# bifurcation/fourq

Hardware: NVIDIA B200
Metric: curve4q_variable_base_dh_scalar_mults_per_s (higher is better)
Workload: dtype u32

## Files before the change

### fourq_b200/csrc/fp.cuh

```cuda
#pragma once
#include "arith.cuh"

struct fp { u32 v[4]; };

struct fpb { u32 b0, b1, b2, b3, e1, e2, e3, d2, d3; };

struct facc { u32 e0, e1, e2, e3, e4, o1, o2, o3, o4, o5; };

struct fpw { u32 w[6]; };

#define FQ_P3 0x7fffffffu

FQ_FN fp fp_set(u32 a0, u32 a1, u32 a2, u32 a3) { fp r; r.v[0] = a0; r.v[1] = a1; r.v[2] = a2; r.v[3] = a3; return r; }
FQ_FN fp fp_zero() { return fp_set(0, 0, 0, 0); }
FQ_FN fp fp_one() { return fp_set(1, 0, 0, 0); }


FQ_FN fp fp_add_loose(const fp& a, const fp& b) {
  fp r;
  r.v[0] = add_cc(a.v[0], b.v[0]); r.v[1] = addc_cc(a.v[1], b.v[1]);
  r.v[2] = addc_cc(a.v[2], b.v[2]); r.v[3] = addc(a.v[3], b.v[3]);
  return r;
}

FQ_FN fp fp_fold1(const fp& x) {
  fp r; u32 t = x.v[3] >> 31;
  r.v[0] = add_cc(x.v[0], t); r.v[1] = addc_cc(x.v[1], 0);
  r.v[2] = addc_cc(x.v[2], 0); r.v[3] = addc(x.v[3] & FQ_P3, 0);
  return r;
}

FQ_FN fp fp_add(const fp& a, const fp& b) { return fp_fold1(fp_add_loose(a, b)); }

FQ_FN fp fp_sub(const fp& a, const fp& b) {
  fp r;
  r.v[0] = sub_cc(a.v[0], b.v[0]); r.v[1] = subc_cc(a.v[1], b.v[1]);
  r.v[2] = subc_cc(a.v[2], b.v[2]); r.v[3] = subc_cc(a.v[3], b.v[3]);
  r.v[0] = subc_cc(r.v[0], 0); r.v[1] = subc_cc(r.v[1], 0);
  r.v[2] = subc_cc(r.v[2], 0); r.v[3] = subc(r.v[3], 0) & FQ_P3;
  return r;
}

FQ_FN fp fp_neg(const fp& a) { return fp_set(~a.v[0], ~a.v[1], ~a.v[2], a.v[3] ^ FQ_P3); }

FQ_FN fp fp_dbl(const fp& a) {
  return fp_set((a.v[0] << 1) | (a.v[3] >> 30), shl_pair(a.v[0], a.v[1], 1), shl_pair(a.v[1], a.v[2], 1),
                shl_pair(a.v[2], a.v[3], 1) & FQ_P3);
}
FQ_FN fp fp_half(const fp& a) {
  return fp_set(shr_pair(a.v[0], a.v[1], 1), shr_pair(a.v[1], a.v[2], 1), shr_pair(a.v[2], a.v[3], 1),
                (a.v[3] >> 1) | ((a.v[0] & 1) << 30));
}

FQ_FN fp fp_canon(const fp& a) {
  u32 allones = a.v[0] & a.v[1] & a.v[2] & (a.v[3] | 0x80000000u);
  u32 m = (allones == 0xffffffffu) ? 0u : 0xffffffffu;
  return fp_set(a.v[0] & m, a.v[1] & m, a.v[2] & m, a.v[3] & m);
}
FQ_FN bool fp_eq_canon(const fp& a, const fp& b) {
  return ((a.v[0] ^ b.v[0]) | (a.v[1] ^ b.v[1]) | (a.v[2] ^ b.v[2]) | (a.v[3] ^ b.v[3])) == 0;
}
FQ_FN bool fp_is_zero(const fp& a) {
  u32 o = a.v[0] | a.v[1] | a.v[2] | a.v[3];
  u32 n = a.v[0] & a.v[1] & a.v[2] & (a.v[3] | 0x80000000u);
  return (o == 0) | (n == 0xffffffffu);
}
FQ_FN fp fp_select(u32 m, const fp& x, const fp& y) {
  return fp_set(y.v[0] ^ (m & (x.v[0] ^ y.v[0])), y.v[1] ^ (m & (x.v[1] ^ y.v[1])),
                y.v[2] ^ (m & (x.v[2] ^ y.v[2])), y.v[3] ^ (m & (x.v[3] ^ y.v[3])));
}
FQ_FN fp fp_from_u128(const fp& x) { return fp_fold1(fp_fold1(x)); }


FQ_FN fpb fp_prep(const fp& b) {
  fpb B;
  B.b0 = b.v[0]; B.b1 = b.v[1]; B.b2 = b.v[2]; B.b3 = b.v[3];
  B.e1 = b.v[1] << 1; B.e2 = b.v[2] << 1; B.e3 = b.v[3] << 1;
  B.d2 = shl_pair(b.v[1], b.v[2], 1); B.d3 = shl_pair(b.v[2], b.v[3], 1);
  return B;
}

FQ_FN void facc_zero(facc& A) { A.e0 = A.e1 = A.e2 = A.e3 = A.e4 = A.o1 = A.o2 = A.o3 = A.o4 = A.o5 = 0; }

template <int K> FQ_FN void facc_init_kp(facc& A) {
  A.e0 = 0; A.e1 = 0u - (1u << (K - 32)); A.e2 = 0xffffffffu; A.e3 = 0xffffffffu; A.e4 = 0;
  A.o1 = 0; A.o2 = 0; A.o3 = 0; A.o4 = 0xffffffffu; A.o5 = (1u << (K - 33)) - 1u;
}

FQ_FN void facc_row0(facc& A, u32 a, u32 v0, u32 v1, u32 v2, u32 v3) {
  mul_wide(A.e0, A.e1, a, v0); mul_wide(A.e2, A.e3, a, v2); A.e4 = 0;
  mul_wide(A.o1, A.o2, a, v1); mul_wide(A.o3, A.o4, a, v3); A.o5 = 0;
}
FQ_FN void facc_row(facc& A, u32 a, u32 v0, u32 v1, u32 v2, u32 v3) {
  A.e0 = mad_lo_cc(a, v0, A.e0); A.e1 = madc_hi_cc(a, v0, A.e1);
  A.e2 = madc_lo_cc(a, v2, A.e2); A.e3 = madc_hi_cc(a, v2, A.e3); A.e4 = addc(A.e4, 0);
  A.o1 = mad_lo_cc(a, v1, A.o1); A.o2 = madc_hi_cc(a, v1, A.o2);
  A.o3 = madc_lo_cc(a, v3, A.o3); A.o4 = madc_hi_cc(a, v3, A.o4); A.o5 = addc(A.o5, 0);
}

template <bool FRESH> FQ_FN void facc_mul(facc& A, const fp& a, const fpb& B) {
  if (FRESH) facc_row0(A, a.v[0], B.b0, B.b1, B.b2, B.b3);
  else facc_row(A, a.v[0], B.b0, B.b1, B.b2, B.b3);
  facc_row(A, a.v[1], B.e3, B.b0, B.b1, B.b2);
  facc_row(A, a.v[2], B.e2, B.d3, B.b0, B.b1);
  facc_row(A, a.v[3], B.e1, B.d2, B.d3, B.b0);
}

FQ_FN fpw facc_merge(const facc& A) {
  fpw r;
  r.w[0] = A.e0; r.w[1] = add_cc(A.e1, A.o1); r.w[2] = addc_cc(A.e2, A.o2); r.w[3] = addc_cc(A.e3, A.o3);
  r.w[4] = addc_cc(A.e4, A.o4); r.w[5] = addc(A.o5, 0);
  return r;
}
FQ_FN fpw fpw_add(const fpw& a, const fpw& b) {
  fpw r;
  r.w[0] = add_cc(a.w[0], b.w[0]); r.w[1] = addc_cc(a.w[1], b.w[1]); r.w[2] = addc_cc(a.w[2], b.w[2]);
  r.w[3] = addc_cc(a.w[3], b.w[3]); r.w[4] = addc_cc(a.w[4], b.w[4]); r.w[5] = addc(a.w[5], b.w[5]);
  return r;
}
FQ_FN fpw fpw_sub(const fpw& a, const fpw& b) {
  fpw r;
  r.w[0] = sub_cc(a.w[0], b.w[0]); r.w[1] = subc_cc(a.w[1], b.w[1]); r.w[2] = subc_cc(a.w[2], b.w[2]);
  r.w[3] = subc_cc(a.w[3], b.w[3]); r.w[4] = subc_cc(a.w[4], b.w[4]); r.w[5] = subc(a.w[5], b.w[5]);
  return r;
}

FQ_FN fp fp_fold(const fpw& x) {
  fp r;
  u32 tlo = shr_pair(x.w[3], x.w[4], 31), thi = shr_pair(x.w[4], x.w[5], 31);
  r.v[0] = add_cc(x.w[0], tlo); r.v[1] = addc_cc(x.w[1], thi);
  r.v[2] = addc_cc(x.w[2], 0); r.v[3] = addc(x.w[3] & FQ_P3, 0);
  u32 top = r.v[3] >> 31;
  r.v[3] &= FQ_P3;
  r.v[0] = add_cc(r.v[0], top); r.v[1] = addc(r.v[1], 0);
  return r;
}

FQ_FN fp fp_mul_prep(const fp& a, const fpb& B) {
  facc A; facc_mul<true>(A, a, B);
  return fp_fold(facc_merge(A));
}
FQ_FN fp fp_mul(const fp& a, const fp& b) { return fp_mul_prep(a, fp_prep(b)); }
FQ_FN fp fp_fold7(u32 w0, u32 w1, u32 w2, u32 w3, u32 w4, u32 w5, u32 w6) {
  fp r;
  u32 t0 = shr_pair(w3, w4, 31), t1 = shr_pair(w4, w5, 31), t2 = shr_pair(w5, w6, 31), t3 = w6 >> 31;
  r.v[0] = add_cc(w0, t0); r.v[1] = addc_cc(w1, t1); r.v[2] = addc_cc(w2, t2); r.v[3] = addc(w3 & FQ_P3, t3);
  u32 top = r.v[3] >> 31;
  r.v[3] &= FQ_P3;
  r.v[0] = add_cc(r.v[0], top); r.v[1] = addc_cc(r.v[1], 0); r.v[2] = addc_cc(r.v[2], 0); r.v[3] = addc(r.v[3], 0);
  return r;
}
FQ_FN fp fp_sqr(const fp& a) {
  const u32 a0 = a.v[0], a1 = a.v[1], a2 = a.v[2], a3 = a.v[3];
  const u32 e1 = a1 << 1, e2 = a2 << 1, e3 = a3 << 1, d2 = shl_pair(a1, a2, 1), d3 = shl_pair(a2, a3, 1);
  u32 E0, E1, E2, E3, E4, E5, E6, O1, O2, O3, O4, O5, O6;
  mul_wide(E0, E1, a0, a0); mul_wide(E2, E3, a0, d2); mul_wide(E4, E5, a1, d3);
  E2 = mad_lo_cc(a1, a1, E2); E3 = madc_hi_cc(a1, a1, E3); E4 = madc_lo_cc(a2, a2, E4); E5 = madc_hi_cc(a2, a2, E5); E6 = addc(0, 0);
  E2 = mad_lo_cc(a3, e3, E2); E3 = madc_hi_cc(a3, e3, E3); E4 = addc_cc(E4, 0); E5 = addc_cc(E5, 0); E6 = addc(E6, 0);
  mul_wide(O1, O2, a0, e1); mul_wide(O3, O4, a0, d3); mul_wide(O5, O6, a2, e3);
  O3 = mad_lo_cc(a1, e2, O3); O4 = madc_hi_cc(a1, e2, O4); O5 = addc_cc(O5, 0); O6 = addc(O6, 0);
  u32 w1 = add_cc(E1, O1), w2 = addc_cc(E2, O2), w3 = addc_cc(E3, O3), w4 = addc_cc(E4, O4), w5 = addc_cc(E5, O5), w6 = addc(E6, O6);
  return fp_fold7(E0, w1, w2, w3, w4, w5, w6);
}

FQ_FN fp fp_nsqr(fp x, int n) {
  FQ_NOUNROLL
  for (int i = 0; i < n; i++) x = fp_sqr(x);
  return x;
}

FQ_FN fp fp_inv(const fp& x) {
  fp x3 = fp_mul(fp_sqr(x), x);
  fp xf = fp_mul(fp_nsqr(x3, 2), x3);
  fp x8 = fp_mul(fp_nsqr(xf, 4), xf);
  fp x16 = fp_mul(fp_nsqr(x8, 8), x8);
  fp x32 = fp_mul(fp_nsqr(x16, 16), x16);
  fp t = fp_mul(fp_nsqr(x32, 32), x32);
  t = fp_mul(fp_nsqr(t, 32), x32);
  t = fp_mul(fp_nsqr(t, 16), x16);
  t = fp_mul(fp_nsqr(t, 8), x8);
  t = fp_mul(fp_nsqr(t, 4), xf);
  t = fp_mul(fp_sqr(t), x);
  return fp_mul(fp_nsqr(t, 2), x);
}

FQ_FN fp fp_invsqrt(const fp& x) {
  fp x3 = fp_mul(fp_sqr(x), x);
  fp xf = fp_mul(fp_nsqr(x3, 2), x3);
  fp x5 = fp_mul(fp_sqr(xf), x);
  fp x10 = fp_mul(fp_nsqr(x5, 5), x5);
  fp x20 = fp_mul(fp_nsqr(x10, 10), x10);
  fp x25 = fp_mul(fp_nsqr(x20, 5), x5);
  fp x50 = fp_mul(fp_nsqr(x25, 25), x25);
  fp x100 = fp_mul(fp_nsqr(x50, 50), x50);
  fp x125 = fp_mul(fp_nsqr(x100, 25), x25);
  return x125;
}
```

### fourq_b200/csrc/fp2.cuh

```cuda
#pragma once
#include "fp.cuh"

struct fp2 { fp re, im; };

struct fp2b { fpb re, im, sum; };

FQ_FN fp2 fp2_set(const fp& re, const fp& im) { fp2 r; r.re = re; r.im = im; return r; }
FQ_FN fp2 fp2_zero() { return fp2_set(fp_zero(), fp_zero()); }
FQ_FN fp2 fp2_one() { return fp2_set(fp_one(), fp_zero()); }

FQ_FN fp2 fp2_add(const fp2& a, const fp2& b) { return fp2_set(fp_add(a.re, b.re), fp_add(a.im, b.im)); }
FQ_FN fp2 fp2_sub(const fp2& a, const fp2& b) { return fp2_set(fp_sub(a.re, b.re), fp_sub(a.im, b.im)); }
FQ_FN fp2 fp2_neg(const fp2& a) { return fp2_set(fp_neg(a.re), fp_neg(a.im)); }
FQ_FN fp2 fp2_conj(const fp2& a) { return fp2_set(a.re, fp_neg(a.im)); }
FQ_FN fp2 fp2_dbl(const fp2& a) { return fp2_set(fp_dbl(a.re), fp_dbl(a.im)); }
FQ_FN fp2 fp2_canon(const fp2& a) { return fp2_set(fp_canon(a.re), fp_canon(a.im)); }
FQ_FN bool fp2_eq_canon(const fp2& a, const fp2& b) { return fp_eq_canon(a.re, b.re) & fp_eq_canon(a.im, b.im); }
FQ_FN bool fp2_eq(const fp2& a, const fp2& b) { return fp2_eq_canon(fp2_canon(a), fp2_canon(b)); }
FQ_FN fp2 fp2_select(u32 m, const fp2& x, const fp2& y) { return fp2_set(fp_select(m, x.re, y.re), fp_select(m, x.im, y.im)); }

#ifdef FQ_FP2_SCHOOLBOOK
FQ_FN fp2b fp2_prep(const fp2& b) {
  fp2b B;
  B.re = fp_prep(b.re); B.im = fp_prep(b.im); B.sum = B.re;
  return B;
}
FQ_FN fp2 fp2_mul_prep(const fp2& a, const fp2b& B) {
  facc A0, A1;
  facc_mul<true>(A0, a.re, B.re); facc_mul<false>(A0, fp_neg(a.im), B.im);
  facc_mul<true>(A1, a.re, B.im); facc_mul<false>(A1, a.im, B.re);
  fp2 r;
  r.re = fp_fold(facc_merge(A0));
  r.im = fp_fold(facc_merge(A1));
  return r;
}
#else
FQ_FN fp2b fp2_prep(const fp2& b) {
  fp2b B;
  B.re = fp_prep(b.re); B.im = fp_prep(b.im); B.sum = fp_prep(fp_add(b.re, b.im));
  return B;
}

FQ_FN fp2 fp2_mul_prep(const fp2& a, const fp2b& B) {
  facc A0, A1, A2;
  facc_init_kp<36>(A0); facc_mul<false>(A0, a.re, B.re);
  facc_mul<true>(A1, a.im, B.im);
  facc_init_kp<38>(A2); facc_mul<false>(A2, fp_add_loose(a.re, a.im), B.sum);
  fpw t0 = facc_merge(A0), t1 = facc_merge(A1), t2 = facc_merge(A2);
  fp2 r;
  r.re = fp_fold(fpw_sub(t0, t1));
  r.im = fp_fold(fpw_sub(fpw_sub(t2, t0), t1));
  return r;
}
#endif
FQ_FN fp2 fp2_mul(const fp2& a, const fp2& b) { return fp2_mul_prep(a, fp2_prep(b)); }

FQ_FN fp2 fp2_sqr(const fp2& a) {
  fp2 r;
  r.re = fp_mul_prep(fp_add_loose(a.re, a.im), fp_prep(fp_sub(a.re, a.im)));
  r.im = fp_mul_prep(fp_add_loose(a.re, a.re), fp_prep(a.im));
  return r;
}

FQ_FN fp2 fp2_inv(const fp2& a) {
  fp n = fp_inv(fp_add(fp_sqr(a.re), fp_sqr(a.im)));
  fpb N = fp_prep(n);
  return fp2_set(fp_mul_prep(a.re, N), fp_mul_prep(fp_neg(a.im), N));
}

#ifdef FQ_HOSTSIM
#define FQ_CALL static inline
#else
#define FQ_CALL static __device__ __noinline__
#endif
FQ_CALL fp2 fp2_mul_c(fp2 a, fp2 b) { return fp2_mul(a, b); }
FQ_CALL fp2 fp2_sqr_c(fp2 a) { return fp2_sqr(a); }
FQ_CALL fp fp_invsqrt_c(fp a) { return fp_invsqrt(a); }
```

### fourq_b200/csrc/point.cuh

```cuda
#pragma once
#include "fp2.cuh"

struct ptR1 { fp2 X, Y, Z, Ta, Tb; };
struct ptR2 { fp2 N, D, E, F; };
struct ptR3p { fp2b N, D, E, F; };

FQ_FN fp2 curve_d() { return fp2_set(fp_set(0x00000142u, 0x00000000u, 0x000000e4u, 0x00000000u), fp_set(0xf1fc0c8du, 0xb3821488u, 0x6657e0fcu, 0x5e472f84u)); }
FQ_FN fp2 curve_2d() { return fp2_set(fp_set(0x00000284u, 0x00000000u, 0x000001c8u, 0x00000000u), fp_set(0xe3f8191bu, 0x67042911u, 0xccafc1f9u, 0x3c8e5f08u)); }
FQ_FN fp2 curve_gx() { return fp2_set(fp_set(0x7b3833aau, 0x286592adu, 0x7c2fb305u, 0x1a347223u), fp_set(0x60ac77f6u, 0x96869fb3u, 0x2878aa9cu, 0x1e1f553fu)); }
FQ_FN fp2 curve_gy() { return fp2_set(fp_set(0x2bcbb287u, 0xb924a246u, 0xa120785au, 0x0e3fee9bu), fp_set(0x844c8b5cu, 0x49a7c344u, 0x630e0242u, 0x6e1c4af8u)); }

FQ_CALL bool pt_on_curve(fp2 x, fp2 y) {
  fp2 x2 = fp2_sqr_c(x), y2 = fp2_sqr_c(y);
  fp2 lhs = fp2_sub(y2, x2);
  fp2 rhs = fp2_add(fp2_one(), fp2_mul_c(fp2_mul_c(curve_d(), x2), y2));
  return fp2_eq(lhs, rhs);
}

FQ_FN ptR1 pt_from_affine(const fp2& x, const fp2& y) { ptR1 P; P.X = x; P.Y = y; P.Z = fp2_one(); P.Ta = x; P.Tb = y; return P; }

FQ_FN ptR2 pt_r1_to_r2(const ptR1& P) {
  ptR2 R;
  R.N = fp2_add(P.X, P.Y); R.D = fp2_sub(P.Y, P.X); R.E = fp2_dbl(P.Z);
  R.F = fp2_mul(fp2_mul(P.Ta, P.Tb), curve_2d());
  return R;
}
FQ_FN ptR3p pt_r1_to_r3p(const ptR1& P) {
  ptR3p R;
  R.N = fp2_prep(fp2_add(P.X, P.Y)); R.D = fp2_prep(fp2_sub(P.Y, P.X)); R.E = fp2_prep(P.Z);
  R.F = fp2_prep(fp2_mul(P.Ta, P.Tb));
  return R;
}
FQ_FN ptR1 pt_r2_to_r4(const ptR2& P) {
  ptR1 Q; Q.X = fp2_sub(P.N, P.D); Q.Y = fp2_add(P.D, P.N); Q.Z = P.E; Q.Ta = fp2_zero(); Q.Tb = fp2_zero();
  return Q;
}
FQ_FN ptR2 pt_r2_cneg(u32 m, const ptR2& P) {
  ptR2 R;
  R.N = fp2_select(m, P.D, P.N); R.D = fp2_select(m, P.N, P.D); R.E = P.E;
  R.F.re = fp_set(P.F.re.v[0] ^ m, P.F.re.v[1] ^ m, P.F.re.v[2] ^ m, P.F.re.v[3] ^ (m & FQ_P3));
  R.F.im = fp_set(P.F.im.v[0] ^ m, P.F.im.v[1] ^ m, P.F.im.v[2] ^ m, P.F.im.v[3] ^ (m & FQ_P3));
  return R;
}

FQ_FN void pt_dbl(ptR1& Q) {
  fp2 A = fp2_sqr(Q.X); FQ_SCHED_FENCE();
  fp2 B = fp2_sqr(Q.Y); FQ_SCHED_FENCE();
  fp2 C = fp2_dbl(fp2_sqr(Q.Z)); FQ_SCHED_FENCE();
  fp2 D = fp2_add(A, B);
  fp2 E = fp2_sub(fp2_sqr(fp2_add(Q.X, Q.Y)), D); FQ_SCHED_FENCE();
  fp2 F = fp2_sub(B, A);
  fp2 G = fp2_sub(C, F);
  fp2b Gp = fp2_prep(G), Fp = fp2_prep(F);
  Q.X = fp2_mul_prep(E, Gp); FQ_SCHED_FENCE();
  Q.Y = fp2_mul_prep(D, Fp); FQ_SCHED_FENCE();
  Q.Z = fp2_mul_prep(F, Gp); FQ_SCHED_FENCE();
  Q.Ta = E; Q.Tb = D;
}

FQ_FN ptR1 pt_add_core(const ptR3p& P, const ptR2& S) {
  fp2 A = fp2_mul_prep(S.D, P.D); FQ_SCHED_FENCE();
  fp2 B = fp2_mul_prep(S.N, P.N); FQ_SCHED_FENCE();
  fp2 C = fp2_mul_prep(S.F, P.F); FQ_SCHED_FENCE();
  fp2 D = fp2_mul_prep(S.E, P.E); FQ_SCHED_FENCE();
  fp2 E = fp2_sub(B, A), F = fp2_sub(D, C), G = fp2_add(D, C), H = fp2_add(B, A);
  fp2b Fp = fp2_prep(F), Gp = fp2_prep(G);
  ptR1 R;
  R.X = fp2_mul_prep(E, Fp); FQ_SCHED_FENCE();
  R.Y = fp2_mul_prep(H, Gp); FQ_SCHED_FENCE();
  R.Z = fp2_mul_prep(G, Fp); FQ_SCHED_FENCE();
  R.Ta = E; R.Tb = H;
  return R;
}
FQ_FN ptR1 pt_add(const ptR1& Q, const ptR2& S) { return pt_add_core(pt_r1_to_r3p(Q), S); }

struct ptR3 { fp2 N, D, E, F; };
#ifdef FQ_SMALL_POINT_OPS
FQ_CALL ptR1 pt_dbl_v(ptR1 Q) {
  fp2 A = fp2_sqr_c(Q.X), B = fp2_sqr_c(Q.Y), C = fp2_dbl(fp2_sqr_c(Q.Z));
  fp2 D = fp2_add(A, B), E = fp2_sub(fp2_sqr_c(fp2_add(Q.X, Q.Y)), D), F = fp2_sub(B, A), G = fp2_sub(C, F);
  ptR1 R; R.X = fp2_mul_c(E, G); R.Y = fp2_mul_c(D, F); R.Z = fp2_mul_c(F, G); R.Ta = E; R.Tb = D;
  return R;
}
#else
FQ_CALL ptR1 pt_dbl_v(ptR1 q) { pt_dbl(q); return q; }
#endif
FQ_FN void pt_dbl_c(ptR1* Q) { *Q = pt_dbl_v(*Q); }
FQ_FN void pt_r1_to_r3_c(ptR3* R, const ptR1* P) {
  R->N = fp2_add(P->X, P->Y); R->D = fp2_sub(P->Y, P->X); R->E = P->Z; R->F = fp2_mul_c(P->Ta, P->Tb);
}
#ifdef FQ_SMALL_POINT_OPS
FQ_CALL ptR1 pt_add_core_v(ptR3 P, ptR2 S) {
  fp2 A = fp2_mul_c(S.D, P.D), B = fp2_mul_c(S.N, P.N), C = fp2_mul_c(S.F, P.F), D = fp2_mul_c(S.E, P.E);
  fp2 E = fp2_sub(B, A), F = fp2_sub(D, C), G = fp2_add(D, C), H = fp2_add(B, A);
  ptR1 R; R.X = fp2_mul_c(E, F); R.Y = fp2_mul_c(H, G); R.Z = fp2_mul_c(G, F); R.Ta = E; R.Tb = H;
  return R;
}
#else
FQ_CALL ptR1 pt_add_core_v(ptR3 P, ptR2 S) {
  ptR3p Pp; Pp.N = fp2_prep(P.N); Pp.D = fp2_prep(P.D); Pp.E = fp2_prep(P.E); Pp.F = fp2_prep(P.F);
  return pt_add_core(Pp, S);
}
#endif
FQ_FN void pt_add_core_c(ptR1* out, const ptR3* P, const ptR2* S) { *out = pt_add_core_v(*P, *S); }
FQ_FN void pt_r1_to_r2_c(ptR2* R, const ptR1* P) {
  R->N = fp2_add(P->X, P->Y); R->D = fp2_sub(P->Y, P->X); R->E = fp2_dbl(P->Z);
  R->F = fp2_mul_c(fp2_mul_c(P->Ta, P->Tb), curve_2d());
}

FQ_FN ptR1 pt_clear_cofactor(const fp2& x, const fp2& y) {
  ptR1 Q = pt_from_affine(x, y);
  ptR2 B; pt_r1_to_r2_c(&B, &Q);
  FQ_NOUNROLL
  for (int i = 0; i < 10; i++) {
    if (i == 1 || i == 6) { ptR3 Q3; pt_r1_to_r3_c(&Q3, &Q); pt_add_core_c(&Q, &Q3, &B); }
    else pt_dbl_c(&Q);
  }
  return Q;
}

FQ_FN void pt_to_affine(const ptR1& P, fp2& x, fp2& y) {
  fp2b Zi = fp2_prep(fp2_inv(P.Z));
  x = fp2_canon(fp2_mul_prep(P.X, Zi)); y = fp2_canon(fp2_mul_prep(P.Y, Zi));
}
```

Baseline: 91.29 million.

## Defer modular reduction in point doubling and addition via wide accumulators

Introduces wide (unreduced) Fp2 multiply and square variants that return 6-word results, biased by multiples of p through facc_init_kp so later subtractions cannot go negative. Point doubling and addition now add and subtract these wide products before a single fold, instead of folding each product and then doing reduced add/sub. This removes several fold and carry-normalisation passes per point operation in exchange for wider intermediates and more live registers, which may cost occupancy.

```diff
diff --git a/fourq_b200/csrc/fp.cuh b/fourq_b200/csrc/fp.cuh
--- a/fourq_b200/csrc/fp.cuh
+++ b/fourq_b200/csrc/fp.cuh
@@ -122,6 +122,13 @@
   fpw r;
   r.w[0] = sub_cc(a.w[0], b.w[0]); r.w[1] = subc_cc(a.w[1], b.w[1]); r.w[2] = subc_cc(a.w[2], b.w[2]);
   r.w[3] = subc_cc(a.w[3], b.w[3]); r.w[4] = subc_cc(a.w[4], b.w[4]); r.w[5] = subc(a.w[5], b.w[5]);
+  return r;
+}
+
+FQ_FN fpw fpw_sub_fp(const fpw& a, const fp& b) {
+  fpw r;
+  r.w[0] = sub_cc(a.w[0], b.v[0]); r.w[1] = subc_cc(a.w[1], b.v[1]); r.w[2] = subc_cc(a.w[2], b.v[2]);
+  r.w[3] = subc_cc(a.w[3], b.v[3]); r.w[4] = subc_cc(a.w[4], 0); r.w[5] = subc(a.w[5], 0);
   return r;
 }
 
diff --git a/fourq_b200/csrc/fp2.cuh b/fourq_b200/csrc/fp2.cuh
--- a/fourq_b200/csrc/fp2.cuh
+++ b/fourq_b200/csrc/fp2.cuh
@@ -55,10 +55,41 @@
 #endif
 FQ_FN fp2 fp2_mul(const fp2& a, const fp2& b) { return fp2_mul_prep(a, fp2_prep(b)); }
 
+struct fp2w { fpw re, im; };
+
+template <int K0, int K2> FQ_FN fp2w fp2_mul_prep_w(const fp2& a, const fp2b& B) {
+  facc A0, A1, A2;
+  facc_init_kp<K0>(A0); facc_mul<false>(A0, a.re, B.re);
+  facc_mul<true>(A1, a.im, B.im);
+  facc_init_kp<K2>(A2); facc_mul<false>(A2, fp_add_loose(a.re, a.im), B.sum);
+  fpw t0 = facc_merge(A0), t1 = facc_merge(A1), t2 = facc_merge(A2);
+  fp2w r;
+  r.re = fpw_sub(t0, t1);
+  r.im = fpw_sub(fpw_sub(t2, t0), t1);
+  return r;
+}
+FQ_FN void fp2w_sum_diff(const fp2w& u, const fp2w& v, fp2& sum, fp2& diff) {
+  sum.re = fp_fold(fpw_add(u.re, v.re)); sum.im = fp_fold(fpw_add(u.im, v.im));
+  diff.re = fp_fold(fpw_sub(u.re, v.re)); diff.im = fp_fold(fpw_sub(u.im, v.im));
+}
+
 FQ_FN fp2 fp2_sqr(const fp2& a) {
   fp2 r;
   r.re = fp_mul_prep(fp_add_loose(a.re, a.im), fp_prep(fp_sub(a.re, a.im)));
   r.im = fp_mul_prep(fp_add_loose(a.re, a.re), fp_prep(a.im));
+  return r;
+}
+
+template <int K, bool TWICE> FQ_FN fp2w fp2_sqr_w(const fp2& a) {
+  const fp d = fp_sub(a.re, a.im);
+  const fpb Bre = fp_prep(TWICE ? fp_dbl(d) : d), Bim = fp_prep(TWICE ? fp_dbl(a.im) : a.im);
+  facc Are, Aim;
+  if constexpr (K == 0) { facc_mul<true>(Are, fp_add_loose(a.re, a.im), Bre); facc_mul<true>(Aim, fp_add_loose(a.re, a.re), Bim); }
+  else {
+    facc_init_kp<K>(Are); facc_mul<false>(Are, fp_add_loose(a.re, a.im), Bre);
+    facc_init_kp<K>(Aim); facc_mul<false>(Aim, fp_add_loose(a.re, a.re), Bim);
+  }
+  fp2w r; r.re = facc_merge(Are); r.im = facc_merge(Aim);
   return r;
 }
 
diff --git a/fourq_b200/csrc/point.cuh b/fourq_b200/csrc/point.cuh
--- a/fourq_b200/csrc/point.cuh
+++ b/fourq_b200/csrc/point.cuh
@@ -44,13 +44,18 @@
 }
 
 FQ_FN void pt_dbl(ptR1& Q) {
-  fp2 A = fp2_sqr(Q.X); FQ_SCHED_FENCE();
-  fp2 B = fp2_sqr(Q.Y); FQ_SCHED_FENCE();
-  fp2 C = fp2_dbl(fp2_sqr(Q.Z)); FQ_SCHED_FENCE();
-  fp2 D = fp2_add(A, B);
-  fp2 E = fp2_sub(fp2_sqr(fp2_add(Q.X, Q.Y)), D); FQ_SCHED_FENCE();
-  fp2 F = fp2_sub(B, A);
-  fp2 G = fp2_sub(C, F);
+  fp2 D, E, F, G;
+  {
+    fp2w A = fp2_sqr_w<0, false>(Q.X); FQ_SCHED_FENCE();
+    fp2w B = fp2_sqr_w<36, false>(Q.Y); FQ_SCHED_FENCE();
+    fp2w_sum_diff(B, A, D, F);
+  }
+  {
+    fp2w S = fp2_sqr_w<38, false>(fp2_add(Q.X, Q.Y)); FQ_SCHED_FENCE();
+    E.re = fp_fold(fpw_sub_fp(S.re, D.re)); E.im = fp_fold(fpw_sub_fp(S.im, D.im));
+    fp2w C = fp2_sqr_w<36, true>(Q.Z); FQ_SCHED_FENCE();
+    G.re = fp_fold(fpw_sub_fp(C.re, F.re)); G.im = fp_fold(fpw_sub_fp(C.im, F.im));
+  }
   fp2b Gp = fp2_prep(G), Fp = fp2_prep(F);
   Q.X = fp2_mul_prep(E, Gp); FQ_SCHED_FENCE();
   Q.Y = fp2_mul_prep(D, Fp); FQ_SCHED_FENCE();
@@ -59,11 +64,17 @@
 }
 
 FQ_FN ptR1 pt_add_core(const ptR3p& P, const ptR2& S) {
-  fp2 A = fp2_mul_prep(S.D, P.D); FQ_SCHED_FENCE();
-  fp2 B = fp2_mul_prep(S.N, P.N); FQ_SCHED_FENCE();
-  fp2 C = fp2_mul_prep(S.F, P.F); FQ_SCHED_FENCE();
-  fp2 D = fp2_mul_prep(S.E, P.E); FQ_SCHED_FENCE();
-  fp2 E = fp2_sub(B, A), F = fp2_sub(D, C), G = fp2_add(D, C), H = fp2_add(B, A);
+  fp2 E, F, G, H;
+  {
+    fp2w A = fp2_mul_prep_w<36, 38>(S.D, P.D); FQ_SCHED_FENCE();
+    fp2w B = fp2_mul_prep_w<38, 40>(S.N, P.N); FQ_SCHED_FENCE();
+    fp2w_sum_diff(B, A, H, E);
+  }
+  {
+    fp2w C = fp2_mul_prep_w<36, 38>(S.F, P.F); FQ_SCHED_FENCE();
+    fp2w D = fp2_mul_prep_w<38, 40>(S.E, P.E); FQ_SCHED_FENCE();
+    fp2w_sum_diff(D, C, G, F);
+  }
   fp2b Fp = fp2_prep(F), Gp = fp2_prep(G);
   ptR1 R;
   R.X = fp2_mul_prep(E, Fp); FQ_SCHED_FENCE();
```

New measurement: 91.71 million, median of 6. About the same (+0.5%).
